# fanmengdan/HD-GNN

Hardware: AMD Instinct MI355X
Metric: training-step commits/sec, glide Ne=200 Nc=74 batch=100; 1/2/4/8 GPU (higher is better)
Workload: dtype f32; 1 GPU; model_2 (HD-GNN/S) train step: fwd+bwd+TF-Adam, glide step=2; launch=hipGraph replay, 4 training steps per graph, ne=200, nc=74, batch_per_gpu=100, global_batch=100, parallelism=dp1

## Files before the change

hd-gnn_amd/csrc/hdgnn.hip:

```cpp
#include <hip/hip_runtime.h>

#include <math.h>
#include <stdint.h>
#include <stdlib.h>

#include <type_traits>

#include "hdgnn.h"
#include "hdgnn_internal.h"
#include "fused_tail.h"

namespace {

using namespace hdg;

constexpr int KK_MID = 5;

#define HDG_DPP_STEP(ctl, n) "v_add_f32_dpp %" #n ", %" #n ", %" #n " " ctl \
  " row_mask:0xf bank_mask:0xf\n\t"
#define HDG_DPP_STEP3(ctl) HDG_DPP_STEP(ctl, 0) HDG_DPP_STEP(ctl, 1) HDG_DPP_STEP(ctl, 2)
#define HDG_DPP_STEP4(ctl) HDG_DPP_STEP3(ctl) HDG_DPP_STEP(ctl, 3)
#define HDG_DPP_STEP5(ctl) HDG_DPP_STEP4(ctl) HDG_DPP_STEP(ctl, 4)
#define HDG_DPP_BLOCK(S) "s_nop 1\n\t" S("row_mirror") S("row_half_mirror") \
  S("quad_perm:[2,3,0,1]") S("quad_perm:[1,0,3,2]")
// ... 760 lines not shown
    b0 += 4 * sb0;
    b1 += 4 * sb1;
  }
  if (k < K) {
    const bool ok = k + q < K;
    const float av = ok ? a[0] : 0.f;
    c0 = __builtin_amdgcn_mfma_f32_16x16x4f32(av, ok ? b0[0] : 0.f, c0, 0, 0, 0);
    c1 = __builtin_amdgcn_mfma_f32_16x16x4f32(av, ok ? b1[0] : 0.f, c1, 0, 0, 0);
  }
  o0 = c0;
  o1 = c1;
}

__device__ __forceinline__ void mfma_tile16x2_r(const float (&av)[HS / 4], const float* pb0,
                                                const int sb0, const float* pb1, const int sb1,
                                                const int lane, f4v& o0, f4v& o1) {
  static_assert(HS % 4 == 0 && HS / 4 == 5, "one 16-step body and one 4-step");
  const int q = lane >> 4;
  const float* b0 = pb0 + q * sb0;
  const float* b1 = pb1 + q * sb1;
  float bv0[HS / 4], bv1[HS / 4];
#pragma unroll
  for (int u = 0; u < HS / 4; ++u) {
    bv0[u] = b0[4 * u * sb0];
    bv1[u] = b1[4 * u * sb1];
  }
  f4v c0 = {0.f, 0.f, 0.f, 0.f}, c1 = c0;
#pragma unroll
  for (int u = 0; u < HS / 4; ++u) {
    c0 = __builtin_amdgcn_mfma_f32_16x16x4f32(av[u], bv0[u], c0, 0, 0, 0);
    c1 = __builtin_amdgcn_mfma_f32_16x16x4f32(av[u], bv1[u], c1, 0, 0, 0);
  }
  __builtin_amdgcn_sched_group_barrier(0x100, 2 * (HS / 4), 0);
  __builtin_amdgcn_sched_group_barrier(0x008, 2 * (HS / 4), 0);
  o0 = c0;
  o1 = c1;
}

struct EntUnit {
  float w0, w1, c0, d;
};
__device__ __forceinline__ EntUnit ent_unit(const float* Ws, int kk) {
  using namespace m2;
  EntUnit e;
  e.w0 = Ws[E1_W1 + kk];
  e.w1 = Ws[E1_W1 + HS + kk];
  const float w2 = Ws[E1_W1 + 2 * HS + kk];
  e.c0 = w2 + Ws[E1_B1 + kk];
  e.d = Ws[E1_W1 + 3 * HS + kk] - w2;
  return e;
}

constexpr int EG_L = HS / 2, EG_N = 6;

template <int ABL = 0>
__device__ __forceinline__ void entity_fwd(const int t, const float* Ws,
                                           const float* xs, const float* xu, const int* cum,
                                           const double* pxd, const int nd,
                                           const int* offr, const int* offc,
                                           const float* xlr, const float* xlc,
                                           const int n0, const int n1, float* Ps,
                                           float* __restrict__ EG, uint2* __restrict__ bq) {
#pragma clang fp contract(off)
  const int sub = t / EG_L, kp = t - sub * EG_L, k0 = 2 * kp;
  const EntUnit ea = ent_unit(Ws, k0 < HS ? k0 : 0), eb = ent_unit(Ws, k0 < HS ? k0 + 1 : 1);
  const f2 w0 = {ea.w0, eb.w0}, w1 = {ea.w1, eb.w1}, c0 = {ea.c0, eb.c0}, dd = {ea.d, eb.d};
  const bool ra[2] = {ea.w1 >= 0.f, eb.w1 >= 0.f}, ca[2] = {ea.w0 >= 0.f, eb.w0 >= 0.f};
  constexpr int NG = NT_MID / EG_L;
  for (int base = n0; base < n1; base += NG) {
    if constexpr (HDG_SETPRIO) __builtin_amdgcn_s_setprio(3);
    const int i = base + sub;
    const bool live = sub < NG && i < n1;
    const int ic = live ? i : 0;
    const float xi = xs[ic];
    const f2 u = __builtin_elementwise_fma((f2){xi, xi}, w0, c0);
    const f2 v = xi * w1;
    int br[2] = {0, 0}, bc[2] = {0, 0};
    for (int s = (ABL & 1) ? 0 : top_pow2(nd); s > 0; s >>= 1) {
#pragma unroll
      for (int h = 0; h < 2; ++h) {
        const float xr = xu[br[h] + s - 1], xc = xu[bc[h] + s - 1];
        const bool fr = (u[h] + xr * w1[h]) > 0.f;
        const bool fc = (fmaf(xc, w0[h], c0[h]) + v[h]) > 0.f;
        br[h] = (fr != ra[h]) ? br[h] + s : br[h];
        bc[h] = (fc != ca[h]) ? bc[h] + s : bc[h];
      }
    }
#pragma unroll
    for (int h = 0; h < 2; ++h) {
      br[h] = br[h] < nd ? br[h] : nd;
      bc[h] = bc[h] < nd ? bc[h] : nd;
    }
    if constexpr (HDG_SETPRIO) __builtin_amdgcn_s_setprio(2);
    float tot[2] = {0.f, 0.f};
    if constexpr (!(ABL & 2)) {
#pragma unroll
      for (int h = 0; h < 2; ++h) {
        const int rlo = ra[h] ? br[h] : 0, rhi = ra[h] ? nd : br[h];
        const int clo = ca[h] ? bc[h] : 0, chi = ca[h] ? nd : bc[h];
        const float sxr = (float)(pxd[rhi] - pxd[rlo]), sxc = (float)(pxd[chi] - pxd[clo]);
        const float nr = (float)(cum[rhi] - cum[rlo]), nc = (float)(cum[chi] - cum[clo]);
        float acc = fmaf(nr, u[h], w1[h] * sxr);
        acc += fmaf(nc, v[h] + c0[h], w0[h] * sxc);
        tot[h] = fmaf(-2.f, relu(u[h] + v[h]), acc);
      }
    }
    f2 sp = {0.f, 0.f};
    const f2 sg = {dd.x >= 0.f ? 1.f : -1.f, dd.y >= 0.f ? 1.f : -1.f};
    const f2 tg = {dd.x >= 0.f ? dd.x : 0.f, dd.y >= 0.f ? dd.y : 0.f};
    const f2 rd = {fabsf(dd.x) >= 0x1p-100f ? 1.f / dd.x : 0.f,
                   fabsf(dd.y) >= 0x1p-100f ? 1.f / dd.y : 0.f};
    auto xsum = [&](const float* xl, int o, const int o1, const f2 ca, const f2 cb) {
      f2 s0 = {0.f, 0.f}, s1 = s0;
      for (; o + 8 <= o1; o += 8) {
        const float4 xa = *reinterpret_cast<const float4*>(xl + o);
        const float4 xb = *reinterpret_cast<const float4*>(xl + o + 4);
        const f2 a0 = {xa.x, xa.y}, a1 = {xa.z, xa.w}, b0 = {xb.x, xb.y}, b1 = {xb.z, xb.w};
        s0 += clamp_fma2_lo(a0, ca, cb);
        s1 += clamp_fma2_hi(a0, ca, cb);
        s0 += clamp_fma2_lo(a1, ca, cb);
        s1 += clamp_fma2_hi(a1, ca, cb);
        s0 += clamp_fma2_lo(b0, ca, cb);
        s1 += clamp_fma2_hi(b0, ca, cb);
        s0 += clamp_fma2_lo(b1, ca, cb);
        s1 += clamp_fma2_hi(b1, ca, cb);
      }
      if (o < o1) {
        const float4 xa = *reinterpret_cast<const float4*>(xl + o);
        const f2 a0 = {xa.x, xa.y}, a1 = {xa.z, xa.w};
        s0 += clamp_fma2_lo(a0, ca, cb);
        s1 += clamp_fma2_hi(a0, ca, cb);
        s0 += clamp_fma2_lo(a1, ca, cb);
        s1 += clamp_fma2_hi(a1, ca, cb);
      }
      sp += s0 + s1;
    };
    xsum(xlr, ((ABL & 4) || !live) ? 0 : offr[ic], ((ABL & 4) || !live) ? 0 : offr[ic + 1],
         sg * w1 * rd, __builtin_elementwise_fma(sg, u, tg) * rd);
    if constexpr (HDG_SETPRIO) __builtin_amdgcn_s_setprio(1);
    xsum(xlc, ((ABL & 8) || !live) ? 0 : offc[ic], ((ABL & 8) || !live) ? 0 : offc[ic + 1],
         sg * w0 * rd, __builtin_elementwise_fma(sg, c0 + v, tg) * rd);
    sp *= dd;
    if (live && kp < EG_L) {
      const float2 P = make_float2(tot[0] + sp.x, tot[1] + sp.y);
      *reinterpret_cast<float2*>(Ps + i * HS + k0) = P;
      *reinterpret_cast<float2*>(EG + i * HS + k0) = P;
      bq[i * EG_L + kp] = make_uint2((uint32_t)br[0] | ((uint32_t)br[1] << 16),
                                     (uint32_t)bc[0] | ((uint32_t)bc[1] << 16));
    }
  }
  if constexpr (HDG_SETPRIO) __builtin_amdgcn_s_setprio(0);
}

template <bool WIDE>
__device__ __forceinline__ void entity_bwd(const int lane, const int wv, const float* Ws,
                                           const float* xs, const int* cum, const double* pxd,
                                           const int nd, const uint2* __restrict__ bq,
                                           const float* rho, const int* offr, const int* offc,
                                           const float* xlr, const float* xlc,
                                           const int n0, const int n1, f2 (&sv)[4]) {
#pragma clang fp contract(off)
  const int sub = lane / EG_L, kp = lane - sub * EG_L, k0 = 2 * kp;
  const EntUnit ea = ent_unit(Ws, k0), eb = ent_unit(Ws, k0 + 1);
  const f2 w0 = {ea.w0, eb.w0}, w1 = {ea.w1, eb.w1}, c0 = {ea.c0, eb.c0}, dd = {ea.d, eb.d};
  const f2 ddS = dd * (f2){STEP_S, STEP_S};
  const bool ra[2] = {ea.w1 >= 0.f, eb.w1 >= 0.f}, ca[2] = {ea.w0 >= 0.f, eb.w0 >= 0.f};
  f2 S0 = {0.f, 0.f}, S1 = S0, S2 = S0, S3 = S0;
  constexpr int NWV = NT_MID / 64;
  int ms = 0;
  for (int base = n0; base + wv < n1; base += EG_N * NWV) {
    if constexpr (HDG_SETPRIO) trip_prio(ms++);
    const int i = base + wv + NWV * sub;
    const bool live = sub < EG_N && i < n1;
    const int ic = live ? i : n0;
    const float xi = xs[ic];
    const f2 u = __builtin_elementwise_fma((f2){xi, xi}, w0, c0);
    const f2 v = xi * w1, x2 = {xi, xi};
    f2 ri = *reinterpret_cast<const f2*>(rho + ic * HS + k0);
    if (!live) ri = (f2){0.f, 0.f};
    const uint2 qb = bq[ic * EG_L + kp];
    f2 b0, b1, b2;
#pragma unroll
    for (int h = 0; h < 2; ++h) {
      const int qr = (int)((qb.x >> (16 * h)) & 0xffffu), qc = (int)((qb.y >> (16 * h)) & 0xffffu);
      const int rlo = ra[h] ? qr : 0, rhi = ra[h] ? nd : qr;
      const int clo = ca[h] ? qc : 0, chi = ca[h] ? nd : qc;
      float nr = (float)(cum[rhi] - cum[rlo]), nc = (float)(cum[chi] - cum[clo]);
      float sxr = (float)(pxd[rhi] - pxd[rlo]), sxc = (float)(pxd[chi] - pxd[clo]);
      if ((u[h] + v[h]) > 0.f) {
        nr -= 1.f;
        nc -= 1.f;
        sxr -= xi;
        sxc -= xi;
      }
      b0[h] = fmaf(xi, nr, sxc);
      b1[h] = fmaf(xi, nc, sxr);
      b2[h] = nr + nc;
    }
    if constexpr (HDG_SETPRIO) trip_prio(ms++);
    f2 sdr = {0.f, 0.f}, sxr = sdr, sdc = sdr, sxc = sdr, b3 = sdr;
    auto rowf = [&](const float xj) {
      const f2 z0 = u + xj * w1;
      const f2 st1 = HDG_STEPF ? stepf2(z0, ddS) : step2(z0 + dd);
      const f2 dm = st1 - step2(z0);
      sdr += dm;
      sxr = __builtin_elementwise_fma((f2){xj, xj}, dm, sxr);
      b3 += st1;
    };
    auto colf = [&](const float xj) {
      const f2 z0 = __builtin_elementwise_fma((f2){xj, xj}, w0, c0) + v;
      const f2 st1 = HDG_STEPF ? stepf2(z0, ddS) : step2(z0 + dd);
      const f2 dm = st1 - step2(z0);
      sdc += dm;
      sxc = __builtin_elementwise_fma((f2){xj, xj}, dm, sxc);
      b3 += st1;
    };
    auto walk = [&](const float* xl, int o, const int o1, auto f) {
      for (; WIDE && o + 16 < o1; o += 16) {
        float4 xv[4];
#pragma unroll
        for (int c = 0; c < 4; ++c) xv[c] = *reinterpret_cast<const float4*>(xl + o + 4 * c);
#pragma unroll
        for (int c = 0; c < 4; ++c) {
          f(xv[c].x);
          f(xv[c].y);
          f(xv[c].z);
          f(xv[c].w);
        }
      }
      for (; o + 4 < o1; o += 4) {
        const float4 xv = *reinterpret_cast<const float4*>(xl + o);
        f(xv.x);
        f(xv.y);
        f(xv.z);
        f(xv.w);
      }
      if (o < o1) {
        const float4 xv = *reinterpret_cast<const float4*>(xl + o);
        f(xv.x);
        if (xv.y == xv.y) f(xv.y);
        if (xv.z == xv.z) f(xv.z);
        if (xv.w == xv.w) f(xv.w);
      }
    };
    walk(xlr, live ? offr[ic] : 0, live ? offr[ic + 1] : 0, rowf);
    if constexpr (HDG_SETPRIO) trip_prio(ms++);
    walk(xlc, live ? offc[ic] : 0, live ? offc[ic + 1] : 0, colf);
    b0 += __builtin_elementwise_fma(x2, sdr, sxc);
    b1 += __builtin_elementwise_fma(x2, sdc, sxr);
    b2 += sdr + sdc;
    S0 = __builtin_elementwise_fma(ri, b0, S0);
    S1 = __builtin_elementwise_fma(ri, b1, S1);
    S2 = __builtin_elementwise_fma(ri, b2, S2);
    S3 = __builtin_elementwise_fma(ri, b3, S3);
  }
  if constexpr (HDG_SETPRIO) __builtin_amdgcn_s_setprio(0);
  sv[0] = S0; sv[1] = S1; sv[2] = S2; sv[3] = S3;
#pragma unroll
  for (int w = 0; w < 4; ++w)
#pragma unroll
    for (int h = 0; h < 2; ++h) {
      float a = sv[w][h];
      a += __shfl_down(a, 3 * EG_L);
      a += __shfl_down(a, EG_L) + __shfl_down(a, 2 * EG_L);
      sv[w][h] = a;
    }
}

__device__ __forceinline__ uint32_t xtag(const uint32_t epoch, const int slot) {
  return (epoch * 8u + (uint32_t)slot) ^ 0xC0DE5A5Au;
}
constexpr int XSLOTS = 4;
constexpr unsigned long long XWAIT = 2000000ull;
typedef uint32_t xu4 __attribute__((ext_vector_type(4)));

__device__ __forceinline__ void xstore(xu4* p, const xu4 w) {
  asm volatile("global_store_dwordx4 %0, %1, off sc0 sc1" ::"v"(p), "v"(w) : "memory");
}
__device__ __forceinline__ xu4 xload(const xu4* p) {
  xu4 w;
  asm volatile("global_load_dwordx4 %0, %1, off sc0 sc1\n\ts_waitcnt vmcnt(0)"
               : "=v"(w) : "v"(p) : "memory");
  return w;
}
__device__ __forceinline__ void pair_send(const float* v, const int n, xu4* __restrict__ out,
                                          const uint32_t tag, const int t) {
  for (int e = t; 2 * e < n; e += NT_MID)
    xstore(out + e, (xu4){__float_as_uint(v[2 * e]), tag, __float_as_uint(v[2 * e + 1]), tag});
}

__device__ __forceinline__ bool pair_recv_add(float* v, const int n, xu4* __restrict__ in,
                                              const uint32_t tag, const int t) {
  bool late = false;
  const unsigned long long t0 = __builtin_amdgcn_s_memrealtime();
  for (int e = t; 2 * e < n; e += NT_MID) {
    xu4 w = xload(in + e);
    while (w.y != tag || w.w != tag) {
      if (__builtin_amdgcn_s_memrealtime() - t0 > XWAIT) { late = true; break; }
      w = xload(in + e);
    }
    v[2 * e] += __uint_as_float(w.x);
    v[2 * e + 1] += __uint_as_float(w.z);
  }
  __syncthreads();
  return late;
}

__device__ __forceinline__ void xch_fault(float* __restrict__ pb, uint32_t* __restrict__ status,
                                       float* __restrict__ probs, float* __restrict__ logits,
                                       const int b, const int Nc, const int rmul,
                                       const int radd, const int t) {
  const float qnan = __builtin_nanf("");
  if (t == 0) pb[m2::NP + HDG_TR_CE] = qnan;
  if (t == 0 && status) xstore1(status, HDG_STATUS_XCH_TIMEOUT);
  const int Nc1 = Nc - 1, Pc = Nc * Nc1;
  const int rows = (Nc - radd + rmul - 1) / rmul;
  const size_t base = (size_t)b * 2 * Pc;
  for (int e = t; e < rows * Nc1; e += NT_MID) {
    const int r = (rmul * (e / Nc1) + radd) * Nc1 + e % Nc1;
    if (probs) { probs[base + r] = qnan; probs[base + Pc + r] = qnan; }
    if (logits) { logits[base + r] = qnan; logits[base + Pc + r] = qnan; }
  }
}

template <int SMAXC, bool TRAIN, bool STAMPS = false, bool SPLIT = false>
__global__ __launch_bounds__(NT_MID) void k_commit_step(
    const float* __restrict__ x, const uint32_t* __restrict__ abits,
    const uint32_t* __restrict__ ybits, const uint32_t* __restrict__ prep,
    const float* __restrict__ Wg, float* __restrict__ Esave, uint16_t* __restrict__ rowq,
    float* __restrict__ gamg, float* __restrict__ part, float* __restrict__ probs,
    float* __restrict__ logits, int Ne, int Nc, float ce_scale,
    unsigned long long* __restrict__ stamps, float* __restrict__ aux,
    const float* __restrict__ bpow, const int B, unsigned long long* __restrict__ xch,
    uint32_t* __restrict__ status, const uint32_t xfault, const int ee_ins,
    const unsigned long long* __restrict__ ncpart, const int ncpt, float* __restrict__ dnout,
    const int ehr_park) {
  using namespace m2;
  constexpr int NC16 = 16 * SMAXC;
  constexpr int CRED = tile_cred_words<SMAXC, KK_MID>();
  extern __shared__ __attribute__((aligned(16))) float lds[];
  const StepLayout L = step_layout(Ne, Nc, SMAXC);
  const PrepLayout PL = prep_layout(Ne, Nc);
  int b, h;
  if constexpr (SPLIT) {
    b = ((blockIdx.x >> 1) & ~7) | (blockIdx.x & 7);
    h = (blockIdx.x >> 3) & 1;
  } else {
    b = blockIdx.x;
    h = 0;
  }
  if (b >= B) return;
  const int rmul = SPLIT ? 2 : 1, radd = h;
  const int prow = SPLIT ? 2 * b + h : b;
  bool xlate = false;
  constexpr int XS = 16 * SMAXC * HS / 2;
  constexpr int XB = XSLOTS * XS;
  xu4* xin = SPLIT ? reinterpret_cast<xu4*>(xch) + (size_t)(2 * b + h) * XB : nullptr;
  xu4* xout = SPLIT ? reinterpret_cast<xu4*>(xch) + (size_t)(2 * b + 1 - h) * XB : nullptr;
  uint32_t* xctr = SPLIT ? reinterpret_cast<uint32_t*>(reinterpret_cast<xu4*>(xch) +
                                                      (size_t)2 * B * XB) + b
                         : nullptr;
  const uint32_t epoch = SPLIT ? *xctr : 0u;
  const uint32_t xsend = h ? xfault : 0u;
  int t = threadIdx.x;
  int lane = t & 63, wv = t >> 6, g = t >> 8, tg = t & 255;
  int mk = t % HS, msl = t / HS;
  const int WC = (Nc + 31) >> 5;
  const int NE4 = (Ne + 3) & ~3;
  const int Pc = Nc * (Nc - 1);
  int nstamp = 0;
#ifndef HDG_STOP_AFTER
#define HDG_STOP_AFTER -1
#endif
  int nphase = 0;
#define MID_STAMP()                                                                     \
  do {                                                                                  \
    if constexpr (STAMPS) {                                                             \
      if (threadIdx.x == 0) stamps[prow * 32 + nstamp] = __builtin_amdgcn_s_memrealtime(); \
      ++nstamp;                                                                         \
    }                                                                                   \
    if constexpr (HDG_STOP_AFTER >= 0) {                                                \
      if (nphase++ == HDG_STOP_AFTER) return;                                           \
    }                                                                                   \
    asm volatile("" : "+v"(t));                                                         \
    lane = t & 63;                                                                      \
    wv = __builtin_amdgcn_readfirstlane(t >> 6);                                        \
    g = __builtin_amdgcn_readfirstlane(t >> 8);                                         \
    tg = t & 255;                                                                       \
    mk = t % HS;                                                                        \
    msl = t / HS;                                                                       \
  } while (0)
  MID_STAMP();
#define WAVE_STAMP(s)                                                                   \
  do {                                                                                  \
    if constexpr (STAMPS) {                                                             \
      if ((threadIdx.x & 63) == 0)                                                      \
        stamps[(size_t)(SPLIT ? 2 * B : B) * 32 + (prow * 16 + (threadIdx.x >> 6)) * 8 + (s)] = \
            __builtin_amdgcn_s_memrealtime();                                           \
    }                                                                                   \
  } while (0)
  float* Ws = lds + L.W;
  float* xs = lds + L.xs;
  float* xps = lds + L.xps;
  float* os = lds + L.os;
  float* dxp = lds + L.dxp;
  float* xu = lds + L.xu;
  int* cum = (int*)(lds + L.cum);
  double* pxd = (double*)(lds + L.pxd);
  int* offr = (int*)(lds + L.offr);
  int* offc = (int*)(lds + L.offc);
  uint32_t* yb = (uint32_t*)(lds + L.yb);
  float* nb = lds + L.nb;
  float* dnb = lds + L.dnb;
  float* dlt = lds + L.misc;
  float* eps = dlt + HS;
  float* cvec = eps + HS;
  float* ysumv = cvec + HS;
  float* s0v = ysumv + HS;
// ... 685 lines not shown
    const f4v c = mfma_tile16_p<true>(rv ? Dal + rr * HS : kzero, rv ? 1 : 0,
                                      mv ? Ws + H1_W1 + m * HS : kzero, mv ? 1 : 0, HS, lane) +
                  mfma_tile16_p<true>(rv ? Dbe + rr * HS : kzero, rv ? 1 : 0,
                                      mv ? Ws + H1_W1 + (4 + m) * HS : kzero, mv ? 1 : 0, HS, lane);
    if (mv) {
      float* dst = m < 2 ? dnb + m : dnc + (m - 2);
#pragma unroll
      for (int q = 0; q < 4; ++q) dst[2 * (row0 + 4 * (lane >> 4) + q)] = c[q];
    }
  }
  if constexpr (DEFER) {
    if (wv >= SMAXC && wv < SMAXC + 8) x_item(8 + wv - SMAXC, lane);
  }
  __syncthreads();
  uint32_t warm[2] = {0u, 0u};
  if constexpr (SPLIT) {
    pair_send(dnb, 2 * Nc, xout + 2 * XS, xtag(epoch, 3) ^ xsend, t);
    if (dnout) pair_send(dnc, 2 * Nc, xout + 2 * XS + Nc, xtag(epoch, 3) ^ xsend, t);
    if (wv >= 4) {
      const int nw = PL.ncst - PL.ks;
      if constexpr (DEFER) {
        static_assert(2 * (NT_MID - 256) * 16 >= 16 * SMAXC * 256, "warm-up: two lines per thread");
#pragma unroll
        for (int u = 0; u < 2; ++u) {
          const int w = (t - 256 + u * (NT_MID - 256)) * 16;
          if (w < nw) warm[u] = pp[PL.ks + w];
        }
      } else {
        uint32_t acc = 0;
        for (int w = (t - 256) * 16; w < nw; w += (NT_MID - 256) * 16) acc ^= pp[PL.ks + w];
        asm volatile("" ::"v"(acc));
      }
    }
  }
  auto dv1_tile = [=](const int w4, const int lane) {
    const int side = w4 >> 1, col0 = (w4 & 1) * 16;
    const float* D = side ? Dbe : Dal;
    const int r = lane & 15, mc = col0 + (lane & 15);
    const float* pa = r < 4 ? nb + r : ((r == 4 && side == 0) ? kone : kzero);
    const f4v c = mfma_tile16_p<true>(pa, r < 4 ? 4 : 0, mc < HS ? D + mc : kzero,
                                      mc < HS ? HS : 0, Nc, lane);
    const int m = col0 + (lane & 15);
    if (m < HS) {
      if (lane < 16) {
#pragma unroll
        for (int q = 0; q < 4; ++q) pb[H1_W1 + (4 * side + q) * HS + m] = c[q];
      } else if (lane < 32 && side == 0) {
        const float dc1 = c[0];
        pb[H1_B1 + m] = dc1;
        pb[H1_W1 + 8 * HS + m] = dc1 - ysumv[m];
        pb[H1_W1 + 9 * HS + m] = ysumv[m];
      }
    }
  };
  if constexpr (DEFER) {
    x_sum(t);
    __syncthreads();
    MID_STAMP();
    if (wv < 4) {
      dv1_tile(wv, lane);
    } else if (wv < 12) {
      cg_tile(wv - 4, lane);
    } else if (wv == 12) {
      if (lane < HS) x_epilogue(lane);
    } else if (wv == NT_MID / 64 - 1) {
      dc2_row(lane);
    }
    if constexpr (SPLIT) asm volatile("" ::"v"(warm[0]), "v"(warm[1]));
  } else {
    if (wv < 4) dv1_tile(wv, lane);
  }
  if constexpr (SPLIT) {
    if constexpr (STAMPS) MID_STAMP();
    xlate |= pair_recv_add(dnb, 2 * Nc, xin + 2 * XS, xtag(epoch, 3), t);
    if (dnout) xlate |= pair_recv_add(dnc, 2 * Nc, xin + 2 * XS + Nc, xtag(epoch, 3), t);
    if (h == 0 && t == 0) *xctr = epoch + 1u;
  } else {
    __syncthreads();
  }
  if (dnout) {
    if (h == 0)
      for (int e = t; e < 4 * Nc; e += NT_MID) {
        const int c = e >> 2, m = e & 3;
        dnout[(size_t)b * 4 * Nc + e] = m < 2 ? dnb[2 * c + m] : dnc[2 * c + m - 2];
      }
    __syncthreads();
  }
  MID_STAMP();

  float* dxpart = U + 3 * NE4 * HS;
  float* xl2 = U + 5 * NE4 * HS;
  const bool lfit2 = xwords <= L.Uwords - 5 * NE4 * HS;
  float4 lv2[LQ];
#pragma unroll
  for (int u = 0; u < LQ; ++u) {
    const int w = 4 * (t + u * NT_MID);
    lv2[u] = (lfit2 && w < xwords) ? *reinterpret_cast<const float4*>(pp + PL.xl + w)
                                   : make_float4(0.f, 0.f, 0.f, 0.f);
  }
  {
    const uint16_t* ks = reinterpret_cast<const uint16_t*>(pp + PL.ks);
    const uint16_t* kt = reinterpret_cast<const uint16_t*>(pp + PL.kt);
    constexpr int NGX = SPLIT ? 8 : NG_MID, TX = NT_MID / NGX;
    const int gx = t / TX, tx = t - gx * TX;
    const int cq = (Nc + NGX - 1) / NGX;
    const int cb0 = gx * cq, cb1 = (cb0 + cq < Nc) ? cb0 + cq : Nc;
    for (int I = nlo + tx; I < nhi; I += TX) {
      float a0 = 0.f, a1 = 0.f;
      for (int c = cb0; c < cb1; ++c) {
        a0 = fmaf(dnb[2 * c], (float)ks[(size_t)c * Ne + I], a0);
        a1 = fmaf(dnb[2 * c + 1], (float)kt[(size_t)c * Ne + I], a1);
      }
      dxpart[gx * NE4 + I] = a0 + a1;
    }
  }
  if (lfit2) {
#pragma unroll
    for (int u = 0; u < LQ; ++u) {
      const int w = 4 * (t + u * NT_MID);
      if (w < xwords) *reinterpret_cast<float4*>(xl2 + w) = lv2[u];
    }
    for (int w = 4 * (t + LQ * NT_MID); w < xwords; w += 4 * NT_MID)
      *reinterpret_cast<float4*>(xl2 + w) = *reinterpret_cast<const float4*>(pp + PL.xl + w);
  }
  __syncthreads();
  MID_STAMP();

  float* dq = U + 2 * NE4 * HS;
  float* dE = U + 3 * NE4 * HS;
  float* hB = U + 4 * NE4 * HS;
  float* rho = hB;
  float* dw2p = Xm;
  for (int i = nlo + t; i < nhi; i += NT_MID) {
    float d = (dxpart[i] + dxpart[NE4 + i]) + (dxpart[2 * NE4 + i] + dxpart[3 * NE4 + i]);
    if constexpr (SPLIT)
      d += (dxpart[4 * NE4 + i] + dxpart[5 * NE4 + i]) + (dxpart[6 * NE4 + i] + dxpart[7 * NE4 + i]);
    dxp[i] = (os[i] > 0.f) ? d : 0.f;
  }
  {
    const float4* s0 = reinterpret_cast<const float4*>(EG);
    const float4* s1 = reinterpret_cast<const float4*>(EbG);
    const float4* s2 = reinterpret_cast<const float4*>(hEG);
    float4* d0 = reinterpret_cast<float4*>(Ps);
    float4* d1 = reinterpret_cast<float4*>(Eb);
    float4* d2 = reinterpret_cast<float4*>(hB);
    for (int e = nlo * HS / 4 + t; e < nhi * HS / 4; e += NT_MID) {
      d0[e] = s0[e];
      d1[e] = s1[e];
      d2[e] = s2[e];
    }
  }
  __syncthreads();
  MID_STAMP();
  for (int rb = (nlo >> 4) + wv; rb <= ((nhi - 1) >> 4); rb += NT_MID / 64) {
    const int row0 = rb * 16;
    const int ir = row0 + (lane & 15);
    const bool rv = ir >= nlo && ir < nhi;
    float dqa[5];
    {
      const int irc = min(max(ir, nlo), nhi - 1), kq = lane >> 4;
      const float d = dxp[irc];
      float hv[5], wq[5];
#pragma unroll
      for (int u = 0; u < 5; ++u) {
        hv[u] = hB[irc * HS + 4 * u + kq];
        wq[u] = Ws[E3_W2 + 4 * u + kq];
      }
#pragma unroll
      for (int u = 0; u < 5; ++u) {
        const float v = (hv[u] > 0.f) ? wq[u] * d : 0.f;
        dqa[u] = rv ? v : 0.f;
      }
      if (rv) {
#pragma unroll
        for (int u = 0; u < 5; ++u) dq[ir * HS + 4 * u + kq] = dqa[u];
      }
    }
    {
      const int r = lane >> 2, kq = lane & 3, i = row0 + r;
      const bool ok = i >= nlo && i < nhi;
      const int ic = min(max(i, nlo), nhi - 1);
      const float dl = dxp[ic], d = ok ? dl : 0.f;
      float hv[6];
#pragma unroll
      for (int j = 0; j < 6; ++j) hv[j] = hB[ic * HS + min(kq + 4 * j, HS - 1)];
      float v[6];
#pragma unroll
      for (int j = 0; j < 6; ++j) {
        const int k = kq + 4 * j;
        v[j] = (ok && k < HS) ? hv[j] * d : (k == HS ? d : 0.f);
      }
#pragma unroll
      for (int j = 0; j < 6; ++j) {
        v[j] += dppf<0x124>(v[j]);
        v[j] += dppf<0x128>(v[j]);
        v[j] = xrow_sum4(v[j]);
      }
      if (r == 0) {
#pragma unroll
        for (int j = 0; j < 6; ++j)
          if (kq + 4 * j <= HS) dw2p[rb * 21 + kq + 4 * j] = v[j];
      }
    }
    {
      f4v cc[2];
      const int m0 = lane & 15, m1 = 16 + (lane & 15);
      mfma_tile16x2_r(dqa, Ws + E3_W1 + (1 + m0) * HS, 1,
                      m1 < HS ? Ws + E3_W1 + (1 + m1) * HS : kzero, m1 < HS ? 1 : 0, lane, cc[0], cc[1]);
#pragma unroll
      for (int cb = 0; cb < 2; ++cb) {
        const int col0 = cb * 16;
        const f4v c = cc[cb];
        const int m = col0 + (lane & 15);
        if (m < HS) {
#pragma unroll
          for (int q = 0; q < 4; ++q) {
            const int i = row0 + 4 * (lane >> 4) + q;
            if (i >= nlo && i < nhi) dE[i * HS + m] = c[q];
          }
        }
      }
    }
    {
      f4v cc[2];
      const int m0 = lane & 15, m1 = 16 + (lane & 15);
      mfma_tile16x2_p(rv ? dE + ir * HS : kzero, rv ? 1 : 0, Ws + E1_W5 + m0 * HS, 1,
                      m1 < HS ? Ws + E1_W5 + m1 * HS : kzero, m1 < HS ? 1 : 0, HS, lane, cc[0], cc[1]);
#pragma unroll
      for (int cb = 0; cb < 2; ++cb) {
        const int col0 = cb * 16;
        const f4v c = cc[cb];
        const int m = col0 + (lane & 15);
        if (m < HS) {
#pragma unroll
          for (int q = 0; q < 4; ++q) {
            const int i = row0 + 4 * (lane >> 4) + q;
            if (i >= nlo && i < nhi) rho[i * HS + m] = c[q];
          }
        }
      }
    }
  }
  __syncthreads();
  if (t < HDG_TRAILER - 2) pb[NP + 2 + t] = 0.f;
  if (t == 2) fsl[prow] = 0.f;
  MID_STAMP();
  if (wv < 4) {
    const int row0 = (wv >> 1) * 16, col0 = (wv & 1) * 16;
    const int lr = row0 + (lane & 15), kc = col0 + (lane & 15);
    const float* pa = lr == 0 ? xs : (lr <= HS ? Eb + lr - 1 : (lr == HS + 1 ? kone : kzero));
    const int sa = lr == 0 ? 1 : (lr <= HS ? HS : 0);
    const f4v c = mfma_tile16_p<true>(pa + nlo * sa, sa, kc < HS ? dq + kc + nlo * HS : kzero,
                                      kc < HS ? HS : 0, nhi - nlo, lane);
    const int k = col0 + (lane & 15);
    if (k < HS) {
#pragma unroll
      for (int q = 0; q < 4; ++q) {
        const int l = row0 + 4 * (lane >> 4) + q;
        if (l <= HS) pb[E3_W1 + l * HS + k] = c[q];
        else if (l == HS + 1) pb[E3_B1 + k] = c[q];
      }
    }
  } else if (wv < 8) {
    const int row0 = ((wv - 4) >> 1) * 16, col0 = ((wv - 4) & 1) * 16;
    const int lr = row0 + (lane & 15), kc = col0 + (lane & 15);
    const f4v c = mfma_tile16_p<true>(lr < HS ? Ps + lr + nlo * HS : (lr == HS ? kone : kzero),
                                      lr < HS ? HS : 0, kc < HS ? dE + kc + nlo * HS : kzero,
                                      kc < HS ? HS : 0, nhi - nlo, lane);
    const int k = col0 + (lane & 15);
    if (k < HS) {
#pragma unroll
      for (int q = 0; q < 4; ++q) {
        const int l = row0 + 4 * (lane >> 4) + q;
        if (l < HS) pb[E1_W5 + l * HS + k] = c[q];
        else if (l == HS) pb[E1_B5 + k] = twoNe1 * c[q];
      }
    }
  } else if (wv == 8 && lane <= HS) {
    float acc = 0.f;
    for (int rb = nlo >> 4; rb <= ((nhi - 1) >> 4); ++rb) acc += dw2p[rb * 21 + lane];
    pb[lane < HS ? E3_W2 + lane : E3_B2] = acc;
  }
  if (t < 4) pb[TH1 + t] = 0.f;
  MID_STAMP();

  WAVE_STAMP(3);
  f2 e2s[4];
  if (lfit2)
    entity_bwd<false>(lane, wv, Ws, xs, cum, pxd, nd, bq, rho, offr, offc, xl2, xl2, nlo, nhi, e2s);
  else
    entity_bwd<true>(lane, wv, Ws, xs, cum, pxd, nd, bq, rho, offr, offc, xlistg, xlistg, nlo, nhi,
                     e2s);
  WAVE_STAMP(2);
  float* red2 = U + NE4 * HS;
  asm volatile("s_waitcnt vmcnt(0)" ::: "memory");
  __syncthreads();
  if (lane < EG_L) {
#pragma unroll
    for (int w = 0; w < 4; ++w) {
      red2[(wv * 4 + w) * HS + 2 * lane] = e2s[w].x;
      red2[(wv * 4 + w) * HS + 2 * lane + 1] = e2s[w].y;
    }
  }
  __syncthreads();
  if (t < 4 * HS) {
    const int w = t / HS, k = t - w * HS;
    float s = 0.f;
    for (int q = 0; q < NT_MID / 64; ++q) s += red2[(q * 4 + w) * HS + k];
    red[w * 32 + k] = s;
  }
  __syncthreads();
  if (t < HS) {
    const float s0 = red[t], s1 = red[32 + t], s2 = red[64 + t], s3 = red[96 + t];
    pb[E1_W1 + t] = s0;
    pb[E1_W1 + HS + t] = s1;
    pb[E1_W1 + 2 * HS + t] = s2 - s3;
    pb[E1_W1 + 3 * HS + t] = s3;
    pb[E1_B1 + t] = s2;
  }
  if (SPLIT && xlate) {
    pb[NP + HDG_TR_CE] = __builtin_nanf("");
    pb[NP + HDG_TR_FAULT] = 1.f;
    fsl[prow] = 1.f;
    if (status) xstore1(status, HDG_STATUS_XCH_TIMEOUT);
  }
  MID_STAMP();
#undef MID_STAMP
#undef WAVE_STAMP
}

__global__ __launch_bounds__(1024) void k_grad_reduce(const float* __restrict__ part, int B,
                                                      int p_begin, int p_end, int shift_at,
                                                      int shift, float* __restrict__ out) {
  __shared__ RedShared sh;
  const int p = p_begin + blockIdx.x * RED_P + (threadIdx.x & (RED_P - 1));
  uint32_t cnt;
  const float g = reduce_commits(part, B, p, p < p_end, sh, cnt);
  if (threadIdx.x >= RED_P || p >= p_end) return;
  float* o = out + (p - p_begin) + (p >= shift_at ? shift : 0);
  if (p == CNT_SLOT && p + 2 < p_end) put_count(o, cnt);
  else if (p < CNT_SLOT || p > CNT_SLOT + 2) o[0] = g;
}

__global__ __launch_bounds__(1024) void k_reduce_adam(const float* __restrict__ part, int B,
                                                      float* __restrict__ params,
                                                      float* __restrict__ mm,
                                                      float* __restrict__ vv,
                                                      float* __restrict__ bpow,
                                                      const float* __restrict__ aux, float lr,
                                                      float inv_pairs, float* __restrict__ stats,
                                                      float* __restrict__ grad, int fault_rows) {
  using namespace m2;
  __shared__ RedShared sh;
  const int p = blockIdx.x * RED_P + (threadIdx.x & (RED_P - 1));
  bool upd = threadIdx.x < RED_P && p < NP;
  const float w = upd ? params[p] : 0.f, m0 = upd ? mm[p] : 0.f, v0 = upd ? vv[p] : 0.f;
  const float lr_t = lr * aux[4], n1 = aux[2], n2 = aux[3];
  bool bad = false;
  for (int r = threadIdx.x; r < fault_rows; r += NT_MID)
    bad |= part[(size_t)fault_rows * NPART + r] != 0.f;
  uint32_t cnt;
  const float g = reduce_commits(part, B, p, p < GRAD_LEN, sh, cnt);
  if (fault_rows > 0 && __syncthreads_or(bad)) upd = false;
  if (threadIdx.x >= RED_P) return;
  if (p == CNT_SLOT) put_count(grad + p, cnt);
  else if (p < CNT_SLOT || (p > CNT_SLOT + 2 && p < GRAD_LEN)) grad[p] = g;
  if (stats && p == CNT_SLOT) put_count(stats + 4, cnt);
  if (stats && p == NP + HDG_TR_FAULT) stats[7] = g;
  if (p == NP) {
    const float ce = g * inv_pairs;
    if (stats) {
      stats[0] = ce;
      stats[1] = aux[1];
      stats[2] = aux[0];
      stats[3] = 10.f * ce + 0.1f * aux[1] + aux[0];
    }
  }
  if (upd) {
    const float b1 = 0.9f, b2 = 0.999f, ep = 1e-8f;
    float gg = g + 0.001f * w;
    if (p >= TH1 && p < TH1 + 2) gg += 0.001f * w / n1;
    if (p >= TH2 && p < TH2 + 2) gg += 0.001f * w / n2;
    float m = m0, v = v0;
    m += (gg - m) * (1.f - b1);
    v += (gg * gg - v) * (1.f - b2);
    mm[p] = m;
    vv[p] = v;
    params[p] = w - lr_t * m / (sqrtf(v) + ep);
  }
  if (blockIdx.x == 0 && threadIdx.x == 0 && upd) {
    bpow[0] = aux[5];
    bpow[1] = aux[6];
  }
}

__global__ __launch_bounds__(1024) void k_adam_tf(float* __restrict__ params,
                                                  float* __restrict__ mm,
                                                  float* __restrict__ vv,
                                                  float* __restrict__ bpow,
                                                  const float* __restrict__ grad, int np,
                                                  float lr, float inv_pairs,
                                                  float* __restrict__ stats) {
  const int TH1 = np - 4, TH2 = np - 2;
  __shared__ float red[16 * 4];
  __shared__ float sh[4];
  const int t = threadIdx.x, lane = t & 63, wv = t >> 6;
  float w[ADAM_PT], g[ADAM_PT], m[ADAM_PT], v[ADAM_PT];
#pragma unroll
  for (int u = 0; u < ADAM_PT; ++u) {
    const int p = t + u * 1024;
    const bool ok = p < np;
    w[u] = ok ? params[p] : 0.f;
    g[u] = ok ? grad[p] : 0.f;
    m[u] = ok ? mm[p] : 0.f;
    v[u] = ok ? vv[p] : 0.f;
  }
  __shared__ float bp[2];
  if (t == 0) { bp[0] = bpow[0]; bp[1] = bpow[1]; }
  const float ce_sum = grad[np + HDG_TR_CE], fault = grad[np + HDG_TR_FAULT];
  float l2 = 0.f, t1 = 0.f, t2 = 0.f;
#pragma unroll
  for (int u = 0; u < ADAM_PT; ++u) {
    const int p = t + u * 1024;
    l2 = fmaf(w[u], w[u], l2);
    if (p >= TH1 && p < TH1 + 2) t1 = fmaf(w[u], w[u], t1);
    if (p >= TH2 && p < TH2 + 2) t2 = fmaf(w[u], w[u], t2);
  }
  l2 = wave_sum(l2);
  t1 = wave_sum(t1);
  t2 = wave_sum(t2);
  if (lane == 0) { red[wv * 4] = l2; red[wv * 4 + 1] = t1; red[wv * 4 + 2] = t2; }
  __syncthreads();
  if (t < 3) {
    float s = 0.f;
    for (int q = 0; q < 16; ++q) s += red[q * 4 + t];
    sh[t] = s;
  }
  __syncthreads();
  const float n1 = sqrtf(sh[1]), n2 = sqrtf(sh[2]);
  const float b1p = bp[0], b2p = bp[1];
  const float lr_t = lr * sqrtf(1.f - b2p) / (1.f - b1p);
  if (t == 0 && stats) {
    const float ce = ce_sum * inv_pairs;
    const float lmap = 0.01f * (n2 + n1);
    const float lpara = 0.0005f * sh[0];
// ... 620 lines not shown
```

Measured before the change: 1.945 million commits/s.

## Overlap entity-backward bracket work with the rho chain on idle waves

Splits the entity backward pass into a rho-independent bracket phase and a rho-dependent accumulation phase. Waves that are not needed for the 16-row dq/dE/rho MFMA chain now compute a window of bracket trips early, while the chain waves run at raised priority. After the barrier, those saved brackets are folded in using rho, and the remaining trips are redistributed across all waves. This hides the bracket cost behind the serial rho chain, at the price of extra live registers and a more complex trip-assignment scheme.

```diff
diff --git a/hd-gnn_amd/csrc/hdgnn.hip b/hd-gnn_amd/csrc/hdgnn.hip
--- a/hd-gnn_amd/csrc/hdgnn.hip
+++ b/hd-gnn_amd/csrc/hdgnn.hip
@@ -936,118 +936,180 @@
   if constexpr (HDG_SETPRIO) __builtin_amdgcn_s_setprio(0);
 }
 
+#ifndef HDG_E2_WIN
+#define HDG_E2_WIN 1
+#endif
+#ifndef HDG_E2_CHAINPRIO
+#define HDG_E2_CHAINPRIO 1
+#endif
+constexpr int E2_WIN = HDG_E2_WIN, E2_NWV = NT_MID / 64;
+__host__ __device__ constexpr int e2_ntrips(int n0, int n1) { return (n1 - n0 + EG_N - 1) / EG_N; }
+__host__ __device__ constexpr int e2_nchain(int n0, int n1) {
+  const int rbs = n1 > n0 ? ((n1 - 1) >> 4) - (n0 >> 4) + 1 : 0;
+  return rbs < E2_NWV ? rbs : E2_NWV;
+}
+__host__ __device__ constexpr int e2_trip(int wv, int k, int n0, int n1, int win) {
+  const int ntrips = e2_ntrips(n0, n1), nchain = e2_nchain(n0, n1), nfree = E2_NWV - nchain;
+  const int nwin = ntrips < win * nfree ? ntrips : win * nfree;
+  if (k < win) {
+    const int tr = (wv - nchain) + k * nfree;
+    return (wv >= nchain && tr < nwin) ? tr : -1;
+  }
+  const int pos = wv >= 9 ? wv - 9 : (wv == 8 ? 7 : wv + 8);
+  const int tr = nwin + pos + (k - win) * E2_NWV;
+  return tr < ntrips ? tr : -1;
+}
+
+struct E2Lane {
+  int sub, kp;
+  f2 w0, w1, c0, dd, ddS;
+  bool ra[2], ca[2];
+};
+__device__ __forceinline__ E2Lane e2_lane(const int lane, const float* Ws) {
+  E2Lane L;
+  L.sub = lane / EG_L;
+  L.kp = lane - L.sub * EG_L;
+  const EntUnit ea = ent_unit(Ws, 2 * L.kp), eb = ent_unit(Ws, 2 * L.kp + 1);
+  L.w0 = (f2){ea.w0, eb.w0};
+  L.w1 = (f2){ea.w1, eb.w1};
+  L.c0 = (f2){ea.c0, eb.c0};
+  L.dd = (f2){ea.d, eb.d};
+  L.ddS = L.dd * (f2){STEP_S, STEP_S};
+  L.ra[0] = ea.w1 >= 0.f; L.ra[1] = eb.w1 >= 0.f;
+  L.ca[0] = ea.w0 >= 0.f; L.ca[1] = eb.w0 >= 0.f;
+  return L;
+}
+__device__ __forceinline__ int e2_node(const E2Lane& L, const int tr, const int n0, const int n1,
+                                       bool& live) {
+  const int i = n0 + EG_N * tr + L.sub;
+  live = L.sub < EG_N && i < n1;
+  return live ? i : n0;
+}
+
+template <bool WIDE, bool PRIO>
+__device__ __forceinline__ void e2_brackets(const E2Lane& L, const int tr, const float* xs,
+                                            const int* cum, const double* pxd, const int nd,
+                                            const uint2* __restrict__ bq, const int* offr,
+                                            const int* offc, const float* xlr, const float* xlc,
+                                            const int n0, const int n1, int& ms, f2 (&b)[4]) {
+#pragma clang fp contract(off)
+  const f2 w0 = L.w0, w1 = L.w1, c0 = L.c0, dd = L.dd, ddS = L.ddS;
+  if constexpr (HDG_SETPRIO && PRIO) trip_prio(ms++);
+  bool live;
+  const int ic = e2_node(L, tr, n0, n1, live);
+  const float xi = xs[ic];
+  const f2 u = __builtin_elementwise_fma((f2){xi, xi}, w0, c0);
+  const f2 v = xi * w1, x2 = {xi, xi};
+  const uint2 qb = bq[ic * EG_L + L.kp];
+  f2 b0, b1, b2;
+#pragma unroll
+  for (int h = 0; h < 2; ++h) {
+    const int qr = (int)((qb.x >> (16 * h)) & 0xffffu), qc = (int)((qb.y >> (16 * h)) & 0xffffu);
+    const int rlo = L.ra[h] ? qr : 0, rhi = L.ra[h] ? nd : qr;
+    const int clo = L.ca[h] ? qc : 0, chi = L.ca[h] ? nd : qc;
+    float nr = (float)(cum[rhi] - cum[rlo]), nc = (float)(cum[chi] - cum[clo]);
+    float sxr = (float)(pxd[rhi] - pxd[rlo]), sxc = (float)(pxd[chi] - pxd[clo]);
+    if ((u[h] + v[h]) > 0.f) {
+      nr -= 1.f;
+      nc -= 1.f;
+      sxr -= xi;
+      sxc -= xi;
+    }
+    b0[h] = fmaf(xi, nr, sxc);
+    b1[h] = fmaf(xi, nc, sxr);
+    b2[h] = nr + nc;
+  }
+  if constexpr (HDG_SETPRIO && PRIO) trip_prio(ms++);
+  f2 sdr = {0.f, 0.f}, sxr = sdr, sdc = sdr, sxc = sdr, b3 = sdr;
+  auto rowf = [&](const float xj) {
+    const f2 z0 = u + xj * w1;
+    const f2 st1 = HDG_STEPF ? stepf2(z0, ddS) : step2(z0 + dd);
+    const f2 dm = st1 - step2(z0);
+    sdr += dm;
+    sxr = __builtin_elementwise_fma((f2){xj, xj}, dm, sxr);
+    b3 += st1;
+  };
+  auto colf = [&](const float xj) {
+    const f2 z0 = __builtin_elementwise_fma((f2){xj, xj}, w0, c0) + v;
+    const f2 st1 = HDG_STEPF ? stepf2(z0, ddS) : step2(z0 + dd);
+    const f2 dm = st1 - step2(z0);
+    sdc += dm;
+    sxc = __builtin_elementwise_fma((f2){xj, xj}, dm, sxc);
+    b3 += st1;
+  };
+  auto walk = [&](const float* xl, int o, const int o1, auto f) {
+    for (; WIDE && o + 16 < o1; o += 16) {
+      float4 xv[4];
+#pragma unroll
+      for (int c = 0; c < 4; ++c) xv[c] = *reinterpret_cast<const float4*>(xl + o + 4 * c);
+#pragma unroll
+      for (int c = 0; c < 4; ++c) {
+        f(xv[c].x);
+        f(xv[c].y);
+        f(xv[c].z);
+        f(xv[c].w);
+      }
+    }
+    for (; o + 4 < o1; o += 4) {
+      const float4 xv = *reinterpret_cast<const float4*>(xl + o);
+      f(xv.x);
+      f(xv.y);
+      f(xv.z);
+      f(xv.w);
+    }
+    if (o < o1) {
+      const float4 xv = *reinterpret_cast<const float4*>(xl + o);
+      f(xv.x);
+      if (xv.y == xv.y) f(xv.y);
+      if (xv.z == xv.z) f(xv.z);
+      if (xv.w == xv.w) f(xv.w);
+    }
+  };
+  walk(xlr, live ? offr[ic] : 0, live ? offr[ic + 1] : 0, rowf);
+  if constexpr (HDG_SETPRIO && PRIO) trip_prio(ms++);
+  walk(xlc, live ? offc[ic] : 0, live ? offc[ic + 1] : 0, colf);
+  b[0] = b0 + __builtin_elementwise_fma(x2, sdr, sxc);
+  b[1] = b1 + __builtin_elementwise_fma(x2, sdc, sxr);
+  b[2] = b2 + (sdr + sdc);
+  b[3] = b3;
+}
+
+__device__ __forceinline__ void e2_accum(const int lane, const int tr, const float* rho,
+                                         const int n0, const int n1, const f2 (&b)[4],
+                                         f2 (&S)[4]) {
+#pragma clang fp contract(off)
+  const int sub = lane / EG_L, kp = lane - sub * EG_L;
+  const int i = n0 + EG_N * tr + sub;
+  const bool live = sub < EG_N && i < n1;
+  f2 ri = *reinterpret_cast<const f2*>(rho + (live ? i : n0) * HS + 2 * kp);
+  if (!live) ri = (f2){0.f, 0.f};
+#pragma unroll
+  for (int w = 0; w < 4; ++w) S[w] = __builtin_elementwise_fma(ri, b[w], S[w]);
+}
+
 template <bool WIDE>
-__device__ __forceinline__ void entity_bwd(const int lane, const int wv, const float* Ws,
-                                           const float* xs, const int* cum, const double* pxd,
-                                           const int nd, const uint2* __restrict__ bq,
-                                           const float* rho, const int* offr, const int* offc,
-                                           const float* xlr, const float* xlc,
-                                           const int n0, const int n1, f2 (&sv)[4]) {
-#pragma clang fp contract(off)
-  const int sub = lane / EG_L, kp = lane - sub * EG_L, k0 = 2 * kp;
-  const EntUnit ea = ent_unit(Ws, k0), eb = ent_unit(Ws, k0 + 1);
-  const f2 w0 = {ea.w0, eb.w0}, w1 = {ea.w1, eb.w1}, c0 = {ea.c0, eb.c0}, dd = {ea.d, eb.d};
-  const f2 ddS = dd * (f2){STEP_S, STEP_S};
-  const bool ra[2] = {ea.w1 >= 0.f, eb.w1 >= 0.f}, ca[2] = {ea.w0 >= 0.f, eb.w0 >= 0.f};
-  f2 S0 = {0.f, 0.f}, S1 = S0, S2 = S0, S3 = S0;
-  constexpr int NWV = NT_MID / 64;
+__device__ __forceinline__ void e2_tail(const int lane, const int wv, const float* Ws,
+                                        const float* xs, const int* cum, const double* pxd,
+                                        const int nd, const uint2* __restrict__ bq,
+                                        const float* rho, const int* offr, const int* offc,
+                                        const float* xl, const int n0, const int n1,
+                                        const int win, f2 (&S)[4]) {
+  const E2Lane L = e2_lane(lane, Ws);
   int ms = 0;
-  for (int base = n0; base + wv < n1; base += EG_N * NWV) {
-    if constexpr (HDG_SETPRIO) trip_prio(ms++);
-    const int i = base + wv + NWV * sub;
-    const bool live = sub < EG_N && i < n1;
-    const int ic = live ? i : n0;
-    const float xi = xs[ic];
-    const f2 u = __builtin_elementwise_fma((f2){xi, xi}, w0, c0);
-    const f2 v = xi * w1, x2 = {xi, xi};
-    f2 ri = *reinterpret_cast<const f2*>(rho + ic * HS + k0);
-    if (!live) ri = (f2){0.f, 0.f};
-    const uint2 qb = bq[ic * EG_L + kp];
-    f2 b0, b1, b2;
+  for (int k = win, tr; (tr = e2_trip(wv, k, n0, n1, win)) >= 0; ++k) {
+    f2 b[4];
+    e2_brackets<WIDE, true>(L, tr, xs, cum, pxd, nd, bq, offr, offc, xl, xl, n0, n1, ms, b);
+    e2_accum(lane, tr, rho, n0, n1, b, S);
+  }
+  if constexpr (HDG_SETPRIO) __builtin_amdgcn_s_setprio(0);
+#pragma unroll
+  for (int w = 0; w < 4; ++w)
 #pragma unroll
     for (int h = 0; h < 2; ++h) {
-      const int qr = (int)((qb.x >> (16 * h)) & 0xffffu), qc = (int)((qb.y >> (16 * h)) & 0xffffu);
-      const int rlo = ra[h] ? qr : 0, rhi = ra[h] ? nd : qr;
-      const int clo = ca[h] ? qc : 0, chi = ca[h] ? nd : qc;
-      float nr = (float)(cum[rhi] - cum[rlo]), nc = (float)(cum[chi] - cum[clo]);
-      float sxr = (float)(pxd[rhi] - pxd[rlo]), sxc = (float)(pxd[chi] - pxd[clo]);
-      if ((u[h] + v[h]) > 0.f) {
-        nr -= 1.f;
-        nc -= 1.f;
-        sxr -= xi;
-        sxc -= xi;
-      }
-      b0[h] = fmaf(xi, nr, sxc);
-      b1[h] = fmaf(xi, nc, sxr);
-      b2[h] = nr + nc;
-    }
-    if constexpr (HDG_SETPRIO) trip_prio(ms++);
-    f2 sdr = {0.f, 0.f}, sxr = sdr, sdc = sdr, sxc = sdr, b3 = sdr;
-    auto rowf = [&](const float xj) {
-      const f2 z0 = u + xj * w1;
-      const f2 st1 = HDG_STEPF ? stepf2(z0, ddS) : step2(z0 + dd);
-      const f2 dm = st1 - step2(z0);
-      sdr += dm;
-      sxr = __builtin_elementwise_fma((f2){xj, xj}, dm, sxr);
-      b3 += st1;
-    };
-    auto colf = [&](const float xj) {
-      const f2 z0 = __builtin_elementwise_fma((f2){xj, xj}, w0, c0) + v;
-      const f2 st1 = HDG_STEPF ? stepf2(z0, ddS) : step2(z0 + dd);
-      const f2 dm = st1 - step2(z0);
-      sdc += dm;
-      sxc = __builtin_elementwise_fma((f2){xj, xj}, dm, sxc);
-      b3 += st1;
-    };
-    auto walk = [&](const float* xl, int o, const int o1, auto f) {
-      for (; WIDE && o + 16 < o1; o += 16) {
-        float4 xv[4];
-#pragma unroll
-        for (int c = 0; c < 4; ++c) xv[c] = *reinterpret_cast<const float4*>(xl + o + 4 * c);
-#pragma unroll
-        for (int c = 0; c < 4; ++c) {
-          f(xv[c].x);
-          f(xv[c].y);
-          f(xv[c].z);
-          f(xv[c].w);
-        }
-      }
-      for (; o + 4 < o1; o += 4) {
-        const float4 xv = *reinterpret_cast<const float4*>(xl + o);
-        f(xv.x);
-        f(xv.y);
-        f(xv.z);
-        f(xv.w);
-      }
-      if (o < o1) {
-        const float4 xv = *reinterpret_cast<const float4*>(xl + o);
-        f(xv.x);
-        if (xv.y == xv.y) f(xv.y);
-        if (xv.z == xv.z) f(xv.z);
-        if (xv.w == xv.w) f(xv.w);
-      }
-    };
-    walk(xlr, live ? offr[ic] : 0, live ? offr[ic + 1] : 0, rowf);
-    if constexpr (HDG_SETPRIO) trip_prio(ms++);
-    walk(xlc, live ? offc[ic] : 0, live ? offc[ic + 1] : 0, colf);
-    b0 += __builtin_elementwise_fma(x2, sdr, sxc);
-    b1 += __builtin_elementwise_fma(x2, sdc, sxr);
-    b2 += sdr + sdc;
-    S0 = __builtin_elementwise_fma(ri, b0, S0);
-    S1 = __builtin_elementwise_fma(ri, b1, S1);
-    S2 = __builtin_elementwise_fma(ri, b2, S2);
-    S3 = __builtin_elementwise_fma(ri, b3, S3);
-  }
-  if constexpr (HDG_SETPRIO) __builtin_amdgcn_s_setprio(0);
-  sv[0] = S0; sv[1] = S1; sv[2] = S2; sv[3] = S3;
-#pragma unroll
-  for (int w = 0; w < 4; ++w)
-#pragma unroll
-    for (int h = 0; h < 2; ++h) {
-      float a = sv[w][h];
+      float a = S[w][h];
       a += __shfl_down(a, 3 * EG_L);
       a += __shfl_down(a, EG_L) + __shfl_down(a, 2 * EG_L);
-      sv[w][h] = a;
+      S[w][h] = a;
     }
 }
 
@@ -2039,99 +2101,134 @@
   }
   __syncthreads();
   MID_STAMP();
-  for (int rb = (nlo >> 4) + wv; rb <= ((nhi - 1) >> 4); rb += NT_MID / 64) {
-    const int row0 = rb * 16;
-    const int ir = row0 + (lane & 15);
-    const bool rv = ir >= nlo && ir < nhi;
-    float dqa[5];
-    {
-      const int irc = min(max(ir, nlo), nhi - 1), kq = lane >> 4;
-      const float d = dxp[irc];
-      float hv[5], wq[5];
-#pragma unroll
-      for (int u = 0; u < 5; ++u) {
-        hv[u] = hB[irc * HS + 4 * u + kq];
-        wq[u] = Ws[E3_W2 + 4 * u + kq];
-      }
-#pragma unroll
-      for (int u = 0; u < 5; ++u) {
-        const float v = (hv[u] > 0.f) ? wq[u] * d : 0.f;
-        dqa[u] = rv ? v : 0.f;
-      }
-      if (rv) {
-#pragma unroll
-        for (int u = 0; u < 5; ++u) dq[ir * HS + 4 * u + kq] = dqa[u];
-      }
-    }
-    {
-      const int r = lane >> 2, kq = lane & 3, i = row0 + r;
-      const bool ok = i >= nlo && i < nhi;
-      const int ic = min(max(i, nlo), nhi - 1);
-      const float dl = dxp[ic], d = ok ? dl : 0.f;
-      float hv[6];
-#pragma unroll
-      for (int j = 0; j < 6; ++j) hv[j] = hB[ic * HS + min(kq + 4 * j, HS - 1)];
-      float v[6];
-#pragma unroll
-      for (int j = 0; j < 6; ++j) {
-        const int k = kq + 4 * j;
-        v[j] = (ok && k < HS) ? hv[j] * d : (k == HS ? d : 0.f);
-      }
-#pragma unroll
-      for (int j = 0; j < 6; ++j) {
-        v[j] += dppf<0x124>(v[j]);
-        v[j] += dppf<0x128>(v[j]);
-        v[j] = xrow_sum4(v[j]);
-      }
-      if (r == 0) {
-#pragma unroll
-        for (int j = 0; j < 6; ++j)
-          if (kq + 4 * j <= HS) dw2p[rb * 21 + kq + 4 * j] = v[j];
-      }
-    }
-    {
-      f4v cc[2];
-      const int m0 = lane & 15, m1 = 16 + (lane & 15);
-      mfma_tile16x2_r(dqa, Ws + E3_W1 + (1 + m0) * HS, 1,
-                      m1 < HS ? Ws + E3_W1 + (1 + m1) * HS : kzero, m1 < HS ? 1 : 0, lane, cc[0], cc[1]);
-#pragma unroll
-      for (int cb = 0; cb < 2; ++cb) {
-        const int col0 = cb * 16;
-        const f4v c = cc[cb];
-        const int m = col0 + (lane & 15);
-        if (m < HS) {
-#pragma unroll
-          for (int q = 0; q < 4; ++q) {
-            const int i = row0 + 4 * (lane >> 4) + q;
-            if (i >= nlo && i < nhi) dE[i * HS + m] = c[q];
+  f2 e2h[E2_WIN > 0 ? E2_WIN : 1][4];
+  const int e2w = lfit2 ? E2_WIN : 0;
+  if (wv >= e2_nchain(nlo, nhi)) {
+    if constexpr (E2_WIN > 0) {
+      if (e2w > 0 && e2_trip(wv, 0, nlo, nhi, e2w) >= 0) {
+        const E2Lane EL = e2_lane(lane, Ws);
+        int ms = 0;
+#pragma unroll
+        for (int k = 0; k < E2_WIN; ++k) {
+          const int tr = e2_trip(wv, k, nlo, nhi, e2w);
+          if (tr < 0) break;
+          e2_brackets<false, false>(EL, tr, xs, cum, pxd, nd, bq, offr, offc, xl2, xl2, nlo, nhi, ms,
+                                    e2h[k]);
+        }
+        WAVE_STAMP(4);
+      }
+    }
+  } else {
+    if constexpr (HDG_SETPRIO && HDG_E2_CHAINPRIO && E2_WIN > 0) __builtin_amdgcn_s_setprio(3);
+    for (int rb = (nlo >> 4) + wv; rb <= ((nhi - 1) >> 4); rb += NT_MID / 64) {
+      const int row0 = rb * 16;
+      const int ir = row0 + (lane & 15);
+      const bool rv = ir >= nlo && ir < nhi;
+      float dqa[5];
+      {
+        const int irc = min(max(ir, nlo), nhi - 1), kq = lane >> 4;
+        const float d = dxp[irc];
+        float hv[5], wq[5];
+#pragma unroll
+        for (int u = 0; u < 5; ++u) {
+          hv[u] = hB[irc * HS + 4 * u + kq];
+          wq[u] = Ws[E3_W2 + 4 * u + kq];
+        }
+#pragma unroll
+        for (int u = 0; u < 5; ++u) {
+          const float v = (hv[u] > 0.f) ? wq[u] * d : 0.f;
+          dqa[u] = rv ? v : 0.f;
+        }
+        if (rv) {
+#pragma unroll
+          for (int u = 0; u < 5; ++u) dq[ir * HS + 4 * u + kq] = dqa[u];
+        }
+      }
+      {
+        const int r = lane >> 2, kq = lane & 3, i = row0 + r;
+        const bool ok = i >= nlo && i < nhi;
+        const int ic = min(max(i, nlo), nhi - 1);
+        const float dl = dxp[ic], d = ok ? dl : 0.f;
+        float hv[6];
+#pragma unroll
+        for (int j = 0; j < 6; ++j) hv[j] = hB[ic * HS + min(kq + 4 * j, HS - 1)];
+        float v[6];
+#pragma unroll
+        for (int j = 0; j < 6; ++j) {
+          const int k = kq + 4 * j;
+          v[j] = (ok && k < HS) ? hv[j] * d : (k == HS ? d : 0.f);
+        }
+#pragma unroll
+        for (int j = 0; j < 6; ++j) {
+          v[j] += dppf<0x124>(v[j]);
+          v[j] += dppf<0x128>(v[j]);
+          v[j] = xrow_sum4(v[j]);
+        }
+        if (r == 0) {
+#pragma unroll
+          for (int j = 0; j < 6; ++j)
+            if (kq + 4 * j <= HS) dw2p[rb * 21 + kq + 4 * j] = v[j];
+        }
+      }
+      {
+        f4v cc[2];
+        const int m0 = lane & 15, m1 = 16 + (lane & 15);
+        mfma_tile16x2_r(dqa, Ws + E3_W1 + (1 + m0) * HS, 1,
+                        m1 < HS ? Ws + E3_W1 + (1 + m1) * HS : kzero, m1 < HS ? 1 : 0, lane, cc[0],
+                        cc[1]);
+#pragma unroll
+        for (int cb = 0; cb < 2; ++cb) {
+          const int col0 = cb * 16;
+          const f4v c = cc[cb];
+          const int m = col0 + (lane & 15);
+          if (m < HS) {
+#pragma unroll
+            for (int q = 0; q < 4; ++q) {
+              const int i = row0 + 4 * (lane >> 4) + q;
+              if (i >= nlo && i < nhi) dE[i * HS + m] = c[q];
+            }
           }
         }
       }
-    }
-    {
-      f4v cc[2];
-      const int m0 = lane & 15, m1 = 16 + (lane & 15);
-      mfma_tile16x2_p(rv ? dE + ir * HS : kzero, rv ? 1 : 0, Ws + E1_W5 + m0 * HS, 1,
-                      m1 < HS ? Ws + E1_W5 + m1 * HS : kzero, m1 < HS ? 1 : 0, HS, lane, cc[0], cc[1]);
-#pragma unroll
-      for (int cb = 0; cb < 2; ++cb) {
-        const int col0 = cb * 16;
-        const f4v c = cc[cb];
-        const int m = col0 + (lane & 15);
-        if (m < HS) {
-#pragma unroll
-          for (int q = 0; q < 4; ++q) {
-            const int i = row0 + 4 * (lane >> 4) + q;
-            if (i >= nlo && i < nhi) rho[i * HS + m] = c[q];
+      {
+        f4v cc[2];
+        const int m0 = lane & 15, m1 = 16 + (lane & 15);
+        mfma_tile16x2_p(rv ? dE + ir * HS : kzero, rv ? 1 : 0, Ws + E1_W5 + m0 * HS, 1,
+                        m1 < HS ? Ws + E1_W5 + m1 * HS : kzero, m1 < HS ? 1 : 0, HS, lane, cc[0],
+                        cc[1]);
+#pragma unroll
+        for (int cb = 0; cb < 2; ++cb) {
+          const int col0 = cb * 16;
+          const f4v c = cc[cb];
+          const int m = col0 + (lane & 15);
+          if (m < HS) {
+#pragma unroll
+            for (int q = 0; q < 4; ++q) {
+              const int i = row0 + 4 * (lane >> 4) + q;
+              if (i >= nlo && i < nhi) rho[i * HS + m] = c[q];
+            }
           }
         }
       }
     }
+    if constexpr (HDG_SETPRIO && HDG_E2_CHAINPRIO && E2_WIN > 0) __builtin_amdgcn_s_setprio(0);
   }
   __syncthreads();
   if (t < HDG_TRAILER - 2) pb[NP + 2 + t] = 0.f;
   if (t == 2) fsl[prow] = 0.f;
   MID_STAMP();
+  f2 e2s[4] = {{0.f, 0.f}, {0.f, 0.f}, {0.f, 0.f}, {0.f, 0.f}};
+  if constexpr (E2_WIN > 0) {
+    if (e2w > 0 && e2_trip(wv, 0, nlo, nhi, e2w) >= 0) {
+      WAVE_STAMP(6);
+#pragma unroll
+      for (int k = 0; k < E2_WIN; ++k) {
+        const int tr = e2_trip(wv, k, nlo, nhi, e2w);
+        if (tr < 0) break;
+        e2_accum(lane, tr, rho, nlo, nhi, e2h[k], e2s);
+      }
+    }
+  }
   if (wv < 4) {
     const int row0 = (wv >> 1) * 16, col0 = (wv & 1) * 16;
     const int lr = row0 + (lane & 15), kc = col0 + (lane & 15);
@@ -2172,12 +2269,10 @@
   MID_STAMP();
 
   WAVE_STAMP(3);
-  f2 e2s[4];
   if (lfit2)
-    entity_bwd<false>(lane, wv, Ws, xs, cum, pxd, nd, bq, rho, offr, offc, xl2, xl2, nlo, nhi, e2s);
+    e2_tail<false>(lane, wv, Ws, xs, cum, pxd, nd, bq, rho, offr, offc, xl2, nlo, nhi, e2w, e2s);
   else
-    entity_bwd<true>(lane, wv, Ws, xs, cum, pxd, nd, bq, rho, offr, offc, xlistg, xlistg, nlo, nhi,
-                     e2s);
+    e2_tail<true>(lane, wv, Ws, xs, cum, pxd, nd, bq, rho, offr, offc, xlistg, nlo, nhi, e2w, e2s);
   WAVE_STAMP(2);
   float* red2 = U + NE4 * HS;
   asm volatile("s_waitcnt vmcnt(0)" ::: "memory");
```

Result: no change. 1.962 million commits/s, median of 6 (+0.9%).
